# yuliangguo/OmniFusion

Hardware: AMD Instinct MI355X
Metric: panoramas/sec at 512x1024 ERP, N=18 256^2 patches; equi2pers+pers2equi GB/s vs HBM peak (higher is better)
Workload: dtype f16x3 (fp16 hi/lo pairs, fp32 accumulate: fp32-class); 1 GPU; cfg2/cfg4 shard: 8 panoramas/GPU/step, 512x1024 ERP, fov 80, nrows 4 (18 patches); full single-pass spherical_fusion forward (confidence=True) at patch size 128 — the only size the reference network exists at (SURVEY 0.1); random-init weights (seed 42); inputs resident in HBM; resample pair at 18x256^2 reported in roofline_resample; per_gpu_batch=8, global_batch=8, parallelism=image-sharded x1, execution=3 forwards in flight per GPU on 3 streams (spherical_fusion.pipelined)

## Files before the change

omnifusion_amd/csrc/omni_conv_sh.hip:

```cpp
#include "omni_conv_sh_common.h"

namespace {

__constant__ float wino_coef[16][4] = {
    {1, 0, 0, 0}, {1, 1, 0, 0}, {1, -1, 0, 0}, {0, -1, 0, 0},
    {1, 0, 1, 0}, {1, 1, 1, 1}, {1, -1, 1, -1}, {0, -1, 0, -1},
    {1, 0, -1, 0}, {1, 1, -1, -1}, {1, -1, -1, 1}, {0, -1, 0, 1},
    {0, 0, -1, 0}, {0, 0, -1, -1}, {0, 0, -1, 1}, {0, 0, 0, 1}};
template <int BM, int BN, int WM, int WN, int NST = 3, int NL = 0, bool PP = false, bool WINO = false, bool X1 = false>
__global__ __launch_bounds__(64 * (WM * WN + NL)) void conv_sh_kernel(ShConvArgs a)
{
    static_assert(!(WINO && X1), "Winograd: f16x3 only");
    static_assert(!PP || (NL > 0 && WM * WN == 8 && NST >= 3), "ping-pong: eight matrix waves (two per SIMD) + loader waves, three stages");
    static_assert(!WINO || (PP && BM / WM == 32 && BN / WN == 32), "Winograd: the ping-pong kernel with 32 x 32 wave tiles");
    constexpr int NW = WM * WN, LW = NL > 0 ? NL : NW, RPP = 8 * LW;
    constexpr int TM = BM / WM / 32, TN = BN / WN / 32;
    constexpr int APASS = BM / RPP, BPASS = BN / RPP, LPS = APASS + BPASS;
    static_assert(APASS >= 1 && BPASS >= 1, "a tile side must cover at least one DMA pass");
    constexpr int A_BYTES = BM * 128, STAGE = (BM + BN) * 128;
    __shared__ __attribute__((aligned(1024))) unsigned char lds[NST * STAGE];
    __shared__ long long cst[OMNI_ABL(32768) ? 256 : 1];
    const bool stamped = OMNI_ABL(32768) && blockIdx.x == 0 && blockIdx.y == 0 && a.ws != nullptr && a.splitk <= 1;
    auto cstamp = [&](int k) { if (OMNI_ABL(32768) && stamped && (threadIdx.x & 63) == 0 && k < 256) cst[k] = clock64(); };
    auto cdump = [&]() { if (OMNI_ABL(32768) && stamped && threadIdx.x == 0) for (int i = 0; i < 256; ++i) reinterpret_cast<long long*>(a.ws)[i] = cst[i]; };
// ... 633 lines not shown
    a.ws = ws;
    a.wt_major = omni_options().conv_wt_major == 2 || (omni_options().conv_wt_major == 1 &&
                 (long long)Cout * conv_sh_ksteps(a) * 128 > (long long)M * H * W * (C1 + C2) * 4) ? 1 : 0;
    a.post = post; a.post_rows = 1; a.wino_th = a.wino_tw = a.wino_pix = 0;
    if (post) {
        if (post_elems == 0 || post_elems % (size_t)Cout || post_elems / (size_t)Cout > 0x7fffffffull)
            OMNI_FAIL(OMNI_ERR_INVALID, "omni_conv2d_sh: the post-activation addend must hold whole rows of Cout channels");
        a.post_rows = (unsigned)(post_elems / (size_t)Cout);
    }
    hipStream_t s = (hipStream_t)stream;
    if (const int rc = conv_sh_launch(conv_sh_plan(a, fmt, post != nullptr, omni_options()), a, (fmt & 8) != 0, s); rc != OMNI_OK) return rc;
    OMNI_HIP(hipGetLastError());
    if (a.splitk > 1 && reduce) {
        const size_t n4 = (size_t)rows * Cout / 4;
        hipLaunchKernelGGL(sh_splitk_reduce_kernel, dim3((unsigned)((n4 + 255) / 256)), dim3(256), 0, s, (const float*)ws, bias, res, dst,
                           n4, Cout, a.splitk, (size_t)rows * Cout, act, a.dst_sh, a.res_f32);
        OMNI_HIP(hipGetLastError());
    }
    return OMNI_OK;
}

extern "C" int omni_conv2d_sh_plan(int fmt, int M, int H, int W, int C1, int C2, int Cout, int KH, int KW, int stride, int pad, int splitk, int has_post,
                                   int* out, int n_out)
{
    if (!out || n_out < 14) OMNI_FAIL(OMNI_ERR_INVALID, "omni_conv2d_sh_plan: needs room for 14 integers");
    ShConvArgs p{};
    if (const int rc = conv_sh_shape(p, M, H, W, C1, C2, Cout, KH, KW, stride, pad, splitk, has_post != 0); rc != OMNI_OK) return rc;
    const ConvShPlan q = conv_sh_plan(p, fmt, has_post != 0, omni_options());
    const int v[14] = {q.family, q.bm, q.bn, q.wm, q.wn, q.nst, q.nl, q.pp, q.th, q.iw, (int)q.grid_x, (int)q.grid_y, q.threads, p.splitk};
    std::copy(v, v + 14, out);
    return OMNI_OK;
}

extern "C" int omni_splitk_reduce_ln512(const float* parts, int nparts, const float* bias, const float* res, float* tok, const float* lg, const float* lb,
                                        float eps, void* y, int fmt, int rows, omni_stream_t stream)
{
    if (!parts || nparts < 1 || !tok || !lg || !lb || !y || rows <= 0) OMNI_FAIL(OMNI_ERR_INVALID, "omni_splitk_reduce_ln512: null pointer or empty input");
    hipStream_t s = (hipStream_t)stream;
    if (fmt & 1) hipLaunchKernelGGL(sh_splitk_reduce_ln512_kernel<true>, dim3((rows + 3) / 4), dim3(256), 0, s, parts, bias, res, tok, lg, lb, y, rows, nparts, (size_t)rows * 512, eps);
    else         hipLaunchKernelGGL(sh_splitk_reduce_ln512_kernel<false>, dim3((rows + 3) / 4), dim3(256), 0, s, parts, bias, res, tok, lg, lb, y, rows, nparts, (size_t)rows * 512, eps);
    OMNI_HIP(hipGetLastError());
    return OMNI_OK;
}

OMNI_SH_OVERFLOW_ACCESSOR(omni_sh_overflow_conv)

extern "C" int omni_sh_overflow(int* flag, int reset)
{
    if (!flag) OMNI_FAIL(OMNI_ERR_INVALID, "omni_sh_overflow: null output");
    OMNI_HIP(hipDeviceSynchronize());
    unsigned v = 0;
    if (omni_sh_overflow_conv(&v, reset) != 0 || omni_sh_overflow_halo(&v, reset) != 0 || omni_sh_overflow_up2(&v, reset) != 0 ||
        omni_sh_overflow_rows(&v, reset) != 0 || omni_sh_overflow_net(&v, reset) != 0 || omni_sh_overflow_pm(&v, reset) != 0 ||
        omni_sh_overflow_halo2(&v, reset) != 0 || omni_sh_overflow_up2_taps(&v, reset) != 0)
        OMNI_FAIL(OMNI_ERR_HIP, "omni_sh_overflow: could not read the device flag");
    *flag = v ? 1 : 0;
    return OMNI_OK;
}

extern "C" int omni_sh_from_f32(const float* src, void* dst, size_t n, omni_stream_t stream)
{
    if (!src || !dst || n % 32) OMNI_FAIL(OMNI_ERR_INVALID, "omni_sh_from_f32: null pointer or n % 32 != 0");
    if (n == 0) return OMNI_OK;
    hipLaunchKernelGGL(sh_from_f32_kernel, dim3((unsigned)((n / 4 + 255) / 256)), dim3(256), 0, (hipStream_t)stream, src, dst, n / 4);
    OMNI_HIP(hipGetLastError());
    return OMNI_OK;
}
extern "C" int omni_sh_to_f32(const void* src, float* dst, size_t n, omni_stream_t stream)
{
    if (!src || !dst || n % 32) OMNI_FAIL(OMNI_ERR_INVALID, "omni_sh_to_f32: null pointer or n % 32 != 0");
    if (n == 0) return OMNI_OK;
    hipLaunchKernelGGL(sh_to_f32_kernel, dim3((unsigned)((n / 4 + 255) / 256)), dim3(256), 0, (hipStream_t)stream, src, dst, n / 4);
    OMNI_HIP(hipGetLastError());
    return OMNI_OK;
}

namespace {

__global__ __launch_bounds__(256) void wino_input_sh_kernel(const void* __restrict__ src, void* __restrict__ V, int M, int H, int W, int C, size_t nt)
{
    const size_t i = (size_t)blockIdx.x * 256 + threadIdx.x;
    const int cq = C >> 2;
    if (i >= nt * cq) return;
    const size_t tl = i / cq;
    const int c = (int)(i - tl * cq) * 4;
    const int tw = W >> 1, th = H >> 1;
    const int m = (int)(tl / (size_t)(th * tw)), rem = (int)(tl - (size_t)m * th * tw), ty = rem / tw, tx = rem - ty * tw;
    f4v d[4][4];
#pragma unroll
    for (int a_ = 0; a_ < 4; ++a_)
#pragma unroll
        for (int b_ = 0; b_ < 4; ++b_) {
            const int y = 2 * ty - 1 + a_, x = 2 * tx - 1 + b_;
            d[a_][b_] = ((unsigned)y < (unsigned)H && (unsigned)x < (unsigned)W) ? act_load4<true>(src, (((size_t)m * H + y) * W + x) * C + c) : (f4v)(0.0f);
        }
    f4v u[4][4];
#pragma unroll
    for (int b_ = 0; b_ < 4; ++b_) { u[0][b_] = d[0][b_] - d[2][b_]; u[1][b_] = d[1][b_] + d[2][b_]; u[2][b_] = d[2][b_] - d[1][b_]; u[3][b_] = d[1][b_] - d[3][b_]; }
#pragma unroll
    for (int xi = 0; xi < 4; ++xi) {
        const f4v v0 = u[xi][0] - u[xi][2], v1 = u[xi][1] + u[xi][2], v2 = u[xi][2] - u[xi][1], v3 = u[xi][1] - u[xi][3];
        act_store4<true>(V, ((size_t)(4 * xi + 0) * nt + tl) * C + c, v0);
        act_store4<true>(V, ((size_t)(4 * xi + 1) * nt + tl) * C + c, v1);
        act_store4<true>(V, ((size_t)(4 * xi + 2) * nt + tl) * C + c, v2);
        act_store4<true>(V, ((size_t)(4 * xi + 3) * nt + tl) * C + c, v3);
    }
}
// ... 43 lines not shown
```

omnifusion_amd/csrc/omni_conv_sh_common.h:

```cpp
#pragma once
#include <stdlib.h>
#include <algorithm>
#include <type_traits>
#include "omni_internal.h"
#include "omni_sh.h"

#ifndef OMNI_CONV_ABL
#define OMNI_CONV_ABL 0
#endif
#define OMNI_ABL(bit) ((OMNI_CONV_ABL & (bit)) != 0)
#ifndef OMNI_PP_PRIO
#define OMNI_PP_PRIO 0
#endif
#ifndef OMNI_G1_PW
#define OMNI_G1_PW 4
#endif

namespace {

typedef float f16v __attribute__((ext_vector_type(16)));
typedef float f4v __attribute__((ext_vector_type(4)));
typedef _Float16 h8v __attribute__((ext_vector_type(8)));
typedef _Float16 h4v __attribute__((ext_vector_type(4)));
typedef _Float16 h2v __attribute__((ext_vector_type(2)));
// ... 152 lines not shown
            }
            if (a.act == OMNI_ACT_RELU) {
#pragma unroll
                for (int e = 0; e < 4; ++e) { v0[e] = fmaxf(v0[e], 0.f); v1[e] = fmaxf(v1[e], 0.f); }
            } else if (a.act == OMNI_ACT_GELU) {
#pragma unroll
                for (int e = 0; e < 4; ++e) { v0[e] = 0.5f * v0[e] * (1.0f + erff(v0[e] * 0.70710678118654752440f)); v1[e] = 0.5f * v1[e] * (1.0f + erff(v1[e] * 0.70710678118654752440f)); }
            }
            if (post) { v0 += pa[kk]; v1 += pb[kk]; }
            h4v h0, l0, h1, l1;
            sh_split4(v0, h0, l0); sh_split4(v1, h1, l1);
            h8v oh, ol;
#pragma unroll
            for (int e = 0; e < 4; ++e) { oh[e] = h0[e]; oh[4 + e] = h1[e]; ol[e] = l0[e]; ol[4 + e] = l1[e]; }
            *reinterpret_cast<h8v*>((unsigned char*)a.dst + off[kk]) = oh;
            *reinterpret_cast<h8v*>((unsigned char*)a.dst + off[kk] + 64) = ol;
        }
    }
}

__device__ __forceinline__ void splitk_finish(f4v v, size_t o, const float* __restrict__ bias, const void* __restrict__ res, void* __restrict__ dst,
                                              int Cout, int act, int dst_sh, int res_f32)
{
    if (bias) v += *reinterpret_cast<const f4v*>(bias + (o % Cout));
    if (res && res_f32) v += *reinterpret_cast<const f4v*>((const float*)res + o);
    else if (res) {
        const unsigned char* rp = (const unsigned char*)res + sh_off(o);
        v += sh_join4(*reinterpret_cast<const h4v*>(rp), *reinterpret_cast<const h4v*>(rp + 64));
    }
    if (act == OMNI_ACT_RELU) { v.x = fmaxf(v.x, 0.f); v.y = fmaxf(v.y, 0.f); v.z = fmaxf(v.z, 0.f); v.w = fmaxf(v.w, 0.f); }
    else if (act == OMNI_ACT_GELU) {
#pragma unroll
        for (int e = 0; e < 4; ++e) v[e] = 0.5f * v[e] * (1.0f + erff(v[e] * 0.70710678118654752440f));
    }
    if (dst_sh) {
        h4v hi, lo; sh_split4(v, hi, lo);
        unsigned char* dp = (unsigned char*)dst + sh_off(o);
        *reinterpret_cast<h4v*>(dp) = hi; *reinterpret_cast<h4v*>(dp + 64) = lo;
    } else {
        *reinterpret_cast<f4v*>((float*)dst + o) = v;
    }
}

constexpr int HT_W = 32, HPW = HT_W + 2;

}

int omni_halo_launch(const void* args, int bn, int th, bool up2, int iw, bool x1, unsigned grid, hipStream_t s);
int omni_conv_pm_launch(const void* args, int bn, bool x1, unsigned grid_x, unsigned grid_y, hipStream_t s);
int omni_sh_overflow_pm(unsigned* out, int reset);
int omni_halo2_launch(const void* args, int iw, bool x1, unsigned grid, hipStream_t s);
int omni_sh_overflow_halo2(unsigned* out, int reset);
int omni_sh_overflow_up2_taps(unsigned* out, int reset);
int omni_sh_overflow_halo(unsigned* out, int reset);
int omni_sh_overflow_up2(unsigned* out, int reset);
int omni_sh_overflow_rows(unsigned* out, int reset);
int omni_sh_overflow_net(unsigned* out, int reset);
```

omnifusion_amd/csrc/omni_conv_up2.hip:

```cpp
#include "omni_conv_sh_common.h"

namespace {

constexpr int HR_PITCH = 36;
struct HeadsArgs { const void* w16; float* hr; };

template <bool HEADS, bool X1 = false>
__global__ __launch_bounds__(HEADS ? 64 * (4 + OMNI_G1_PW) : 512) void conv3x3_up2_g1_kernel(ShConvArgs a, int ntiles, HeadsArgs hd)
{
    constexpr int BN = 32, TH = 4, NW = 4, RPP = 8 * NW;
    constexpr int PW = HEADS ? OMNI_G1_PW : 4, CPT = 32 / PW;
    constexpr int HPX = (TH + 2) * HPW, HA_INSTR = (HPX * 8 + 63) / 64, HA_BYTES = HA_INSTR * 1024;
    constexpr int BROWS = 3 * BN, BPASS = (BROWS + RPP - 1) / RPP, B_BYTES = BROWS * 128, W_OFF = 2 * HA_BYTES;
    __shared__ __attribute__((aligned(1024))) unsigned char lds[2 * HA_BYTES + 3 * B_BYTES];
    constexpr int ST_N = 40, ST_K = 5;
    __shared__ long long stamps[OMNI_ABL(32768) ? 2 * ST_N * ST_K : 1];
    auto stamp = [&](int who, int it, int k) { if (OMNI_ABL(32768) && blockIdx.x == 0 && it < ST_N && (threadIdx.x & 63) == 0) stamps[(who * ST_N + it) * ST_K + k] = clock64(); };

    const int t = threadIdx.x, lane = t & 63;
    const int wave = __builtin_amdgcn_readfirstlane(t >> 6);
    const bool consumer = wave < NW;
    const int tw = a.W / HT_W, th = a.H / TH, per_img = tw * th;
    const int xcd = blockIdx.x & 7, lb = blockIdx.x >> 3, nlb = gridDim.x >> 3;
    const int per = (ntiles + 7) >> 3, t_end = min(ntiles, (xcd + 1) * per);
// ... 271 lines not shown

extern "C" int omni_conv3x3_up2_sh_f16x3(const void* src, const void* wt16, const float* bias, void* dst, int fmt,
                                         int M, int Hl, int Wl, int C, int Cout, int act, omni_stream_t stream)
{
    if (!src || !wt16 || !dst) OMNI_FAIL(OMNI_ERR_INVALID, "omni_conv3x3_up2_sh: null pointer");
    if (M <= 0 || Hl <= 0 || Wl <= 0 || C <= 0 || C % 32 || Cout <= 0 || Cout % 32) OMNI_FAIL(OMNI_ERR_INVALID, "omni_conv3x3_up2_sh: bad shape (channels must be multiples of 32)");
    const int H = 2 * Hl, W = 2 * Wl;
    if (W % HT_W || H % 4) OMNI_FAIL(OMNI_ERR_UNSUPPORTED, "omni_conv3x3_up2_sh: the output must be a multiple of 4 rows x 32 columns");
    if ((long long)M * H * W >= (1ll << 31) || (long long)Cout * 9 * C * 4 >= (1ll << 31))
        OMNI_FAIL(OMNI_ERR_UNSUPPORTED, "omni_conv3x3_up2_sh: tensor too large for 32-bit indices");
    ShConvArgs a;
    a.src1 = src; a.src2 = nullptr; a.wt = wt16; a.bias = bias; a.res = nullptr; a.dst = dst; a.dst_sh = fmt & 1; a.res_f32 = 0;
    a.dbg = 0; a.noxcd = omni_options().conv_noxcd; a.wt_major = 0; a.epi_lds = omni_options().conv_epi_lds && !(fmt & 4);
#ifdef OMNI_DEBUG_BUILD
    a.dbg = omni_debug_bits("OMNI_CONV_DBG");
#endif
    a.M = M; a.H = H; a.W = W; a.C1 = C; a.C2 = 0; a.Cout = Cout; a.KH = 3; a.KW = 3; a.stride = 1; a.pad = 1; a.act = act;
    a.Ho = H; a.Wo = W; a.rows = M * H * W; a.splitk = 1; a.ws = nullptr; a.post = nullptr; a.post_rows = 1; a.wino_th = a.wino_tw = a.wino_pix = 0;
    const int grid = M * (H / 4) * (W / HT_W);
    const bool x1 = (fmt & 8) != 0;
    if (C == 32 && Cout == 32 && omni_options().conv_up2_persist) {
        const dim3 g1(grid < 256 ? (grid + 7) / 8 * 8 : 256);
        if (x1) hipLaunchKernelGGL((conv3x3_up2_g1_kernel<false, true>), g1, dim3(512), 0, (hipStream_t)stream, a, grid, HeadsArgs{nullptr, nullptr});
        else    hipLaunchKernelGGL(conv3x3_up2_g1_kernel<false>, g1, dim3(512), 0, (hipStream_t)stream, a, grid, HeadsArgs{nullptr, nullptr});
        OMNI_HIP(hipGetLastError());
        return OMNI_OK;
    }
    const bool bn64 = Cout % 64 == 0 && !((fmt & 4) && omni_options().conv_halo_up2_bn_lat == 32);
    const int bn = bn64 ? 64 : 32;
    if (const int rc = omni_halo_launch(&a, bn, 4, true, 0, x1, grid * (Cout / bn), (hipStream_t)stream); rc != OMNI_OK) return rc;
    OMNI_HIP(hipGetLastError());
    return OMNI_OK;
}

extern "C" size_t omni_up2_heads_scratch_bytes(int M, int P)
{
    if (M <= 0 || P <= 0 || P % 32) return 0;
    return (size_t)M * (P / 4) * (P / 32) * 4 * 6 * HR_PITCH * sizeof(float);
}
template <bool X1>
static int up2_heads_impl(const void* src, const void* wt16, const float* bias, const void* heads_w16f, float bias_pred, float bias_weight,
                          float* scratch, size_t scratch_bytes, float* out_a, float* out_c, int M, int P, int confidence, omni_stream_t stream)
{
    if (!src || !wt16 || !heads_w16f || !scratch || !out_a) OMNI_FAIL(OMNI_ERR_INVALID, "omni_conv3x3_up2_heads_sh: null pointer");
    if (M <= 0 || P <= 0 || P % 32) OMNI_FAIL(OMNI_ERR_INVALID, "omni_conv3x3_up2_heads_sh: the patch size must be a multiple of 32");
    if (scratch_bytes < omni_up2_heads_scratch_bytes(M, P)) OMNI_FAIL(OMNI_ERR_INVALID, "omni_conv3x3_up2_heads_sh: scratch too small (omni_up2_heads_scratch_bytes)");
    if ((long long)M * P * P >= (1ll << 31)) OMNI_FAIL(OMNI_ERR_UNSUPPORTED, "omni_conv3x3_up2_heads_sh: tensor too large for 32-bit indices");
    ShConvArgs a;
    a.src1 = src; a.src2 = nullptr; a.wt = wt16; a.bias = bias; a.res = nullptr; a.dst = nullptr; a.dst_sh = 0; a.res_f32 = 0;
    a.dbg = 0; a.noxcd = omni_options().conv_noxcd; a.wt_major = 0; a.epi_lds = 0;
    a.M = M; a.H = P; a.W = P; a.C1 = 32; a.C2 = 0; a.Cout = 32; a.KH = 3; a.KW = 3; a.stride = 1; a.pad = 1; a.act = OMNI_ACT_RELU;
    a.Ho = P; a.Wo = P; a.rows = M * P * P; a.splitk = 1; a.ws = nullptr; a.post = nullptr; a.post_rows = 1; a.wino_th = a.wino_tw = a.wino_pix = 0;
    const int grid = M * (P / 4) * (P / HT_W);
    hipLaunchKernelGGL((conv3x3_up2_g1_kernel<true, X1>), dim3(grid < 256 ? (grid + 7) / 8 * 8 : 256), dim3(64 * (4 + OMNI_G1_PW)), 0, (hipStream_t)stream, a, grid, HeadsArgs{heads_w16f, scratch});
    OMNI_HIP(hipGetLastError());
    const size_t n = (size_t)M * P * P / 4;
    hipLaunchKernelGGL(heads_finish_kernel, dim3((unsigned)((n + 255) / 256)), dim3(256), 0, (hipStream_t)stream, (const float*)scratch, bias_pred, bias_weight,
                       out_a, out_c, M, P, confidence);
    OMNI_HIP(hipGetLastError());
    return OMNI_OK;
}
extern "C" int omni_conv3x3_up2_heads_sh_f16x3(const void* src, const void* wt16, const float* bias, const void* heads_w16f, float bias_pred, float bias_weight,
                                               float* scratch, size_t scratch_bytes, float* out_a, float* out_c, int M, int P, int confidence, omni_stream_t stream)
{
    return up2_heads_impl<false>(src, wt16, bias, heads_w16f, bias_pred, bias_weight, scratch, scratch_bytes, out_a, out_c, M, P, confidence, stream);
}
extern "C" int omni_conv3x3_up2_heads_sh_f16x1(const void* src, const void* wt16, const float* bias, const void* heads_w16f, float bias_pred, float bias_weight,
                                               float* scratch, size_t scratch_bytes, float* out_a, float* out_c, int M, int P, int confidence, omni_stream_t stream)
{
    return up2_heads_impl<true>(src, wt16, bias, heads_w16f, bias_pred, bias_weight, scratch, scratch_bytes, out_a, out_c, M, P, confidence, stream);
}

extern "C" int omni_heads_pack_f16x3(const float* w_host, void* dst_host)
{
    if (!w_host || !dst_host) OMNI_FAIL(OMNI_ERR_INVALID, "omni_heads_pack: null pointer");
    _Float16* o = (_Float16*)dst_host;
    for (int kc = 0; kc < 2; ++kc)
        for (int lane = 0; lane < 64; ++lane)
            for (int e = 0; e < 8; ++e) {
                const int r = lane & 31, h = lane >> 5, g = r >> 3, hh = (r >> 2) & 1, dxi = r & 3;
                float w = 0.0f;
                if (g < 3 && dxi < 3) {
                    const int pair = g + 3 * hh, dy = pair / 2, head = pair % 2, ch = 16 * kc + 8 * (e >> 2) + 4 * h + (e & 3);
                    w = w_host[(head * 9 + dy * 3 + dxi) * 32 + ch];
                }
                const _Float16 hi = (w < 6.103515625e-05f && w > -6.103515625e-05f) ? (_Float16)0.0f : (_Float16)w;
                o[(kc * 64 + lane) * 8 + e] = hi;
                o[((2 + kc) * 64 + lane) * 8 + e] = (_Float16)((w - (float)hi) * 2048.0f);
            }
    return OMNI_OK;
}
```

omnifusion_amd/csrc/omni_geometry.hip:

```cpp
#include <math.h>
#include <stdlib.h>
#include <string.h>
#include <mutex>
#include <vector>
#include <memory>

#include "omni_internal.h"

static thread_local std::string g_err;
void omni_set_error(const std::string& msg) { g_err = msg; }
extern "C" const char* omni_last_error(void) { return g_err.c_str(); }
extern "C" int omni_version(void) { return OMNI_VERSION; }

namespace {
struct OptName { const char* name; const char* env; int OmniOptions::* field; int dflt; };
const OptName kOpts[] = {
    {"conv_sh_tile", "OMNI_CONV_SH_TILE", &OmniOptions::conv_sh_tile, -1},
    {"conv_nohalo", "OMNI_CONV_NOHALO", &OmniOptions::conv_nohalo, 0},
    {"conv_halo_th", "OMNI_CONV_HALO_TH", &OmniOptions::conv_halo_th, 4},
    {"conv_big_blocks", "OMNI_CONV_BIG_BLOCKS", &OmniOptions::conv_big_blocks, 128},
    {"conv_halo_bn_lat", "OMNI_CONV_HALO_BN_LAT", &OmniOptions::conv_halo_bn_lat, 32},
    {"conv_deep_loaders", "OMNI_CONV_DEEP_LOADERS", &OmniOptions::conv_deep_loaders, 1},
    {"conv_halo_up2_bn_lat", "OMNI_CONV_HALO_UP2_BN_LAT", &OmniOptions::conv_halo_up2_bn_lat, 64},
    {"conv_halo_bn", "OMNI_CONV_HALO_BN", &OmniOptions::conv_halo_bn, 64},
    {"conv_img", "OMNI_CONV_IMG", &OmniOptions::conv_img, 1},
    {"conv_nodeep", "OMNI_CONV_NODEEP", &OmniOptions::conv_nodeep, 0},
    {"conv_pingpong", "OMNI_CONV_PINGPONG", &OmniOptions::conv_pingpong, 1},
    {"conv_pm", "OMNI_CONV_PM", &OmniOptions::conv_pm, 1},
    {"conv_noxcd", "OMNI_CONV_NOXCD", &OmniOptions::conv_noxcd, 0},
    {"conv_wt_major", "OMNI_CONV_WT_MAJOR", &OmniOptions::conv_wt_major, 1},
    {"conv_stem_pc", "OMNI_CONV_STEM_PC", &OmniOptions::conv_stem_pc, 1},
    {"conv_epi_lds", "OMNI_CONV_EPI_LDS", &OmniOptions::conv_epi_lds, 1},
    {"conv_up2_persist", "OMNI_CONV_UP2_PERSIST", &OmniOptions::conv_up2_persist, 1},
    {"splitk_max", "OMNI_SPLITK_MAX", &OmniOptions::splitk_max, 0},
    {"e2p_gather", "OMNI_E2P_GATHER", &OmniOptions::e2p_gather, 0},
    {"e2p_notab", "OMNI_E2P_NOTAB", &OmniOptions::e2p_notab, 0},
    {"e2p_verbose", "OMNI_E2P_VERBOSE", &OmniOptions::e2p_verbose, 0},
    {"e2p_bwd_simple", "OMNI_E2P_BWD_SIMPLE", &OmniOptions::e2p_bwd_simple, 0},
    {"p2e_bwd_simple", "OMNI_P2E_BWD_SIMPLE", &OmniOptions::p2e_bwd_simple, 0},
    {"bwd_table_mb", "OMNI_BWD_TABLE_MB", &OmniOptions::bwd_table_mb, 1024},
    {"bwd_wide", "OMNI_BWD_WIDE", &OmniOptions::bwd_wide, 1},
    {"bwd_lmax", "OMNI_BWD_LMAX", &OmniOptions::bwd_lmax, 0},
    {"bwd_chunk", "OMNI_BWD_CHUNK", &OmniOptions::bwd_chunk, 0},
    {"p2e_gather", "OMNI_P2E_GATHER", &OmniOptions::p2e_gather, 0},
    {"e2p_nbuf", "OMNI_E2P_NBUF", &OmniOptions::e2p_nbuf, 0},
    {"e2p_slot_kb", "OMNI_E2P_SLOT_KB", &OmniOptions::e2p_slot_kb, 6},
    {"e2p_tile_h", "OMNI_E2P_TILE_H", &OmniOptions::e2p_tile_h, 0},
    {"e2p_ref_lds", "OMNI_E2P_REF_LDS", &OmniOptions::e2p_ref_lds, 1},
    {"e2p_store", "OMNI_E2P_STORE", &OmniOptions::e2p_store, 1},
    {"e2p_slots", "OMNI_E2P_SLOTS", &OmniOptions::e2p_slots, 0},
    {"e2p_split", "OMNI_E2P_SPLIT", &OmniOptions::e2p_split, 0},
    {"e2p_full", "OMNI_E2P_FULL", &OmniOptions::e2p_full, -1},
    {"e2p_fb_planes", "OMNI_E2P_FB_PLANES", &OmniOptions::e2p_fb_planes, 0},
    {"e2p_fb_pos", "OMNI_E2P_FB_POS", &OmniOptions::e2p_fb_pos, 0},
    {"e2p_region", "OMNI_E2P_REGION", &OmniOptions::e2p_region, 0},
    {"p2e_band", "OMNI_P2E_BAND", &OmniOptions::p2e_band, 0},
    {"p2e_nbuf", "OMNI_P2E_NBUF", &OmniOptions::p2e_nbuf, 0},
    {"p2e_lds_kb", "OMNI_P2E_LDS_KB", &OmniOptions::p2e_lds_kb, 0},
    {"p2e_planes", "OMNI_P2E_PLANES", &OmniOptions::p2e_planes, 0},
    {"p2e_walk", "OMNI_P2E_WALK", &OmniOptions::p2e_walk, 1},
    {"p2e_tile8", "OMNI_P2E_TILE8", &OmniOptions::p2e_tile8, 1},
    {"p2e_store", "OMNI_P2E_STORE", &OmniOptions::p2e_store, 1},
    {"fv_bwd_lds", "OMNI_FV_BWD_LDS", &OmniOptions::fv_bwd_lds, 1},
    {"geom_cache_max", "OMNI_GEOM_CACHE_MAX", &OmniOptions::geom_cache_max, 16},
    {"chamfer_split", "OMNI_CHAMFER_SPLIT", &OmniOptions::chamfer_split, 1},
    {"augment_lut", "OMNI_AUGMENT_LUT", &OmniOptions::augment_lut, 1},
    {"conv_halo2", "OMNI_CONV_HALO2", &OmniOptions::conv_halo2, 1},
    {"conv_wgrad_rows", "OMNI_CONV_WGRAD_ROWS", &OmniOptions::conv_wgrad_rows, 0},
};
}

OmniOptions& omni_options()
{
    static OmniOptions o = [] {
        OmniOptions v;
        for (const OptName& k : kOpts) {
            const char* e = getenv(k.env);
            v.*(k.field) = e ? (*e ? atoi(e) : 1) : k.dflt;
        }
        return v;
    }();
    return o;
}

int omni_num_cus()
{
// ... 250 lines not shown
```

omnifusion_amd/csrc/omni_internal.h:

```cpp
#pragma once
#include <mutex>
#include <hip/hip_runtime.h>
#include <hip/hip_fp16.h>
#include <stdint.h>
#include <string>
#include <vector>

#include "../../include/omnifusion.h"

#define OMNI_MAX_PATCH 46
#define OMNI_WAVE 64

void omni_set_error(const std::string& msg);
#define OMNI_FAIL(code, msg) do { omni_set_error(msg); return (code); } while (0)
#define OMNI_HIP(expr) do { hipError_t e_ = (expr); if (e_ != hipSuccess) {                   \
        omni_set_error(std::string(#expr) + ": " + hipGetErrorString(e_)); return OMNI_ERR_HIP; } } while (0)

struct OmniOptions {
    int conv_sh_tile;
    int conv_nohalo;
    int conv_halo_th;
    int conv_halo_bn_lat;
    int conv_halo_up2_bn_lat;
    int conv_deep_loaders;
    int conv_big_blocks;
    int conv_halo_bn;
    int conv_img;
    int conv_nodeep;
    int conv_pingpong;
    int conv_pm;
    int conv_noxcd;
    int conv_wt_major;
    int conv_stem_pc;
    int conv_epi_lds;
    int conv_up2_persist;
    int splitk_max;
    int e2p_gather;
    int e2p_notab;
    int e2p_verbose;
    int e2p_bwd_simple;
    int p2e_bwd_simple;
    int p2e_gather;
    int e2p_nbuf;
    int e2p_store;
    int e2p_slots;
    int e2p_split;
    int e2p_full;
    int e2p_fb_planes;
    int e2p_region;
    int e2p_fb_pos;
    int e2p_ref_lds;
    int e2p_tile_h;
    int e2p_slot_kb;
    int p2e_band;
    int p2e_lds_kb;
    int p2e_nbuf;
    int p2e_planes;
    int p2e_store;
    int p2e_tile8;
    int p2e_walk;
    int bwd_wide;
    int bwd_chunk;
    int bwd_lmax;
    int bwd_table_mb;
    int fv_bwd_lds;
    int geom_cache_max;
    int chamfer_split;
    int augment_lut;
    int conv_halo2;
    int conv_wgrad_rows;
};
OmniOptions& omni_options();
int omni_num_cus();

#ifdef OMNI_DEBUG_BUILD
#define OMNI_DBG(a, bit) (((a).dbg & (bit)) != 0)
int omni_debug_bits(const char* env_name);
long long* omni_debug_trace_buf();
#else
#define OMNI_DBG(a, bit) false
#endif

struct PatchTab {
    int   N;
    float lam0[OMNI_MAX_PATCH];
    float slam[OMNI_MAX_PATCH];
    float clam[OMNI_MAX_PATCH];
    float sphi[OMNI_MAX_PATCH];
// ... 94 lines not shown
```

omnifusion_amd/isa.py:

```python
import os
import re
import subprocess
import sys
import tempfile

LLVM = os.environ.get("OMNI_LLVM_BIN", "/opt/rocm/lib/llvm/bin")
TARGET = "hipv4-amdgcn-amd-amdhsa--gfx950"
FORBIDDEN = re.compile(r"\bv_pk_(mul|add|fma)_f32\b")
COUNTED = ("e2p_box_kernel", "p2e_lds_kernel", "p2e_walk_kernel", "e2p_ref_kernel", "up2_taps_fused_kernel")
HOT = ("conv_sh_kernel", "conv3x3_halo_sh_kernel", "conv3x3_up2_g1_kernel", "stem_f16x3_pc_kernel", "heads_kernel", "maxpool_kernel",
       "layernorm512_kernel", "attention_kernel", "upsample_sh8_kernel", "halo2_sh_kernel")
HOST_ONLY = ("omni_png.o", "omni_geometry.o")


def _device_object(obj, tmp):
    fat = os.path.join(tmp, "fat.bin")
    co = os.path.join(tmp, "dev.co")
    r = subprocess.run([os.path.join(LLVM, "llvm-objcopy"), "--dump-section", f".hip_fatbin={fat}", obj, os.path.join(tmp, "copy.o")],
                       stderr=subprocess.DEVNULL)
    if r.returncode != 0 or not os.path.exists(fat) or os.path.getsize(fat) == 0:
        return None
    subprocess.check_call([os.path.join(LLVM, "clang-offload-bundler"), "--unbundle", "--type=o", f"--input={fat}",
                           f"--targets={TARGET}", f"--output={co}"])
    return co


def disassemble(obj):
    with tempfile.TemporaryDirectory() as tmp:
        co = _device_object(obj, tmp)
        if co is None:
            return ""
        return subprocess.check_output([os.path.join(LLVM, "llvm-objdump"), "-d", "--mcpu=gfx950", co]).decode()


def kernel_meta(obj):
    with tempfile.TemporaryDirectory() as tmp:
        co = _device_object(obj, tmp)
        if co is None:
            return []
        txt = subprocess.check_output([os.path.join(LLVM, "llvm-readelf"), "--notes", co]).decode()
    out, cur = [], None
    keys = {".vgpr_count": "vgpr", ".agpr_count": "agpr", ".sgpr_count": "sgpr", ".group_segment_fixed_size": "lds",
            ".private_segment_fixed_size": "scratch", ".vgpr_spill_count": "vgpr_spill", ".sgpr_spill_count": "sgpr_spill",
            ".name": "name"}
    for line in txt.splitlines():
        m = re.match(r"^  - \.(\w+):\s*(\S+)\s*$", line)
        if m:
            cur = {}
            out.append(cur)
            line = "    ." + m.group(1) + ": " + m.group(2)
        m = re.match(r"^    (\.\w+):\s*(\S+)\s*$", line)
        if m and cur is not None and m.group(1) in keys:
            v = m.group(2)
            cur[keys[m.group(1)]] = v if m.group(1) == ".name" else int(v)
    return [k for k in out if "name" in k]


def demangle(names):
    try:
        p = subprocess.run([os.path.join(LLVM, "llvm-cxxfilt")], input="\n".join(names).encode(), stdout=subprocess.PIPE, check=True)
        return p.stdout.decode().splitlines()
    except Exception:
# ... 70 lines not shown
```

Baseline: 4475 panoramas/s.

## Add persistent tap-first up2 conv+heads kernel computing conv before upsampling

Adds a new persistent kernel for the final upsample-by-2 3x3 conv plus prediction heads at patch size 128. It applies each 3x3 tap's channel mix at the low 64x64 resolution with MFMA, then does the bilinear upsample separably (vertical, then horizontal) through LDS. The heads 1x1 projection is fused on the parked output. This aims to cut the conv arithmetic by doing the matmuls at a quarter of the pixels, at the cost of a complex LDS schedule, many barriers, and a one-block-per-CU occupancy. The path is on by default through a new option and falls back to the old kernel when pointers are misaligned or the size is not 128.

```diff
diff --git a/omnifusion_amd/csrc/omni_conv_sh.hip b/omnifusion_amd/csrc/omni_conv_sh.hip
--- a/omnifusion_amd/csrc/omni_conv_sh.hip
+++ b/omnifusion_amd/csrc/omni_conv_sh.hip
@@ -709,7 +709,8 @@
     unsigned v = 0;
     if (omni_sh_overflow_conv(&v, reset) != 0 || omni_sh_overflow_halo(&v, reset) != 0 || omni_sh_overflow_up2(&v, reset) != 0 ||
         omni_sh_overflow_rows(&v, reset) != 0 || omni_sh_overflow_net(&v, reset) != 0 || omni_sh_overflow_pm(&v, reset) != 0 ||
-        omni_sh_overflow_halo2(&v, reset) != 0 || omni_sh_overflow_up2_taps(&v, reset) != 0)
+        omni_sh_overflow_halo2(&v, reset) != 0 || omni_sh_overflow_up2_taps(&v, reset) != 0 ||
+        omni_sh_overflow_up2_heads_taps(&v, reset) != 0)
         OMNI_FAIL(OMNI_ERR_HIP, "omni_sh_overflow: could not read the device flag");
     *flag = v ? 1 : 0;
     return OMNI_OK;
diff --git a/omnifusion_amd/csrc/omni_conv_sh_common.h b/omnifusion_amd/csrc/omni_conv_sh_common.h
--- a/omnifusion_amd/csrc/omni_conv_sh_common.h
+++ b/omnifusion_amd/csrc/omni_conv_sh_common.h
@@ -228,6 +228,8 @@
 int omni_halo2_launch(const void* args, int iw, bool x1, unsigned grid, hipStream_t s);
 int omni_sh_overflow_halo2(unsigned* out, int reset);
 int omni_sh_overflow_up2_taps(unsigned* out, int reset);
+int omni_up2_heads_taps_launch(const void* src, const void* wt16, const float* bias, const void* heads_w16f, float* hr, int M, hipStream_t s);
+int omni_sh_overflow_up2_heads_taps(unsigned* out, int reset);
 int omni_sh_overflow_halo(unsigned* out, int reset);
 int omni_sh_overflow_up2(unsigned* out, int reset);
 int omni_sh_overflow_rows(unsigned* out, int reset);
diff --git a/omnifusion_amd/csrc/omni_conv_up2.hip b/omnifusion_amd/csrc/omni_conv_up2.hip
--- a/omnifusion_amd/csrc/omni_conv_up2.hip
+++ b/omnifusion_amd/csrc/omni_conv_up2.hip
@@ -347,8 +347,14 @@
     a.M = M; a.H = P; a.W = P; a.C1 = 32; a.C2 = 0; a.Cout = 32; a.KH = 3; a.KW = 3; a.stride = 1; a.pad = 1; a.act = OMNI_ACT_RELU;
     a.Ho = P; a.Wo = P; a.rows = M * P * P; a.splitk = 1; a.ws = nullptr; a.post = nullptr; a.post_rows = 1; a.wino_th = a.wino_tw = a.wino_pix = 0;
     const int grid = M * (P / 4) * (P / HT_W);
-    hipLaunchKernelGGL((conv3x3_up2_g1_kernel<true, X1>), dim3(grid < 256 ? (grid + 7) / 8 * 8 : 256), dim3(64 * (4 + OMNI_G1_PW)), 0, (hipStream_t)stream, a, grid, HeadsArgs{heads_w16f, scratch});
-    OMNI_HIP(hipGetLastError());
+    const bool taps = !X1 && P == 128 && omni_options().conv_up2_heads_taps == 1 &&
+                      !((uintptr_t)src % 16 || (uintptr_t)wt16 % 16 || (uintptr_t)bias % 16 || (uintptr_t)heads_w16f % 16 || (uintptr_t)scratch % 16);
+    if (taps) {
+        if (const int rc = omni_up2_heads_taps_launch(src, wt16, bias, heads_w16f, scratch, M, (hipStream_t)stream); rc != OMNI_OK) return rc;
+    } else {
+        hipLaunchKernelGGL((conv3x3_up2_g1_kernel<true, X1>), dim3(grid < 256 ? (grid + 7) / 8 * 8 : 256), dim3(64 * (4 + OMNI_G1_PW)), 0, (hipStream_t)stream, a, grid, HeadsArgs{heads_w16f, scratch});
+        OMNI_HIP(hipGetLastError());
+    }
     const size_t n = (size_t)M * P * P / 4;
     hipLaunchKernelGGL(heads_finish_kernel, dim3((unsigned)((n + 255) / 256)), dim3(256), 0, (hipStream_t)stream, (const float*)scratch, bias_pred, bias_weight,
                        out_a, out_c, M, P, confidence);
diff --git a/omnifusion_amd/csrc/omni_conv_up2_heads_taps.hip b/omnifusion_amd/csrc/omni_conv_up2_heads_taps.hip
--- /dev/null
+++ b/omnifusion_amd/csrc/omni_conv_up2_heads_taps.hip
@@ -0,0 +1,287 @@
+#include <stdint.h>
+#include "omni_conv_sh_common.h"
+
+namespace {
+
+constexpr int HR_PITCH = 36;
+
+struct HeadsTapsArgs {
+    const void* src;
+    const void* wt;
+    const float* bias;
+    const void* hw16;
+    float* hr;
+    int nbands;
+};
+
+constexpr int WL = 64, HL = 64, ROWS = 4, SROWS = ROWS + 2, NPX = SROWS * WL, NF = NPX / 32;
+constexpr int TAP_BYTES = 32 * 128, W_BYTES = 9 * TAP_BYTES, CH_BYTES = NPX * 128, ROW_BYTES = WL * 128;
+constexpr int BANDS_PER_IMG = HL / ROWS;
+
+__host__ __device__ constexpr int tap_at(int s) { return 3 * (s % 3) + s / 3; }
+
+__global__ __launch_bounds__(512, 1) void up2_heads_taps_kernel(HeadsTapsArgs a)
+{
+    __shared__ __attribute__((aligned(1024))) unsigned char lds[W_BYTES + 2 * CH_BYTES];
+    static_assert(sizeof(lds) <= 160 * 1024 && NF == 12 && 4 * 128 * 128 <= 2 * CH_BYTES, "one block per CU; half a band's SH rows fit the two chunks");
+
+    const int t = threadIdx.x, lane = t & 63;
+    const int wave = __builtin_amdgcn_readfirstlane(t >> 6);
+    const int xcd = blockIdx.x & 7, lb = blockIdx.x >> 3, nlb = gridDim.x >> 3;
+    const int per = (a.nbands + 7) >> 3, b_end = min(a.nbands, (xcd + 1) * per);
+    int bandid = xcd * per + lb;
+    if (bandid >= b_end) return;
+
+    {
+        const rsrc_t rsw = make_rsrc(a.wt, (size_t)32 * 9 * 128);
+#pragma unroll
+        for (int k = 0; k < 5; ++k) {
+            const int n = wave + 8 * k;
+            if (n < 36) {
+                const int tp = n >> 2, d = (n & 3) * 4 + (lane >> 4), pw = (lane & 15) ^ d, row = 2 * d + (pw >> 3);
+                dma16(rsw, lds + n * 1024, ((row * 9 + tp) * 8 + (pw & 7)) * 16, 0);
+            }
+        }
+    }
+    const int wfo = ((lane & 31) >> 1) * 256 + ((((lane & 1) * 8 + (lane >> 5)) ^ ((lane & 31) >> 1)) * 16);
+
+    auto frag = [&](int fi) { return fi == 0 || wave >= 4 ? wave : wave + 8; };
+    h8v xh[2][2], xl[2][2];
+    auto load_x = [&](int bid) {
+        const int m = bid / BANDS_PER_IMG, sbase = (bid - m * BANDS_PER_IMG) * ROWS - 1;
+#pragma unroll
+        for (int fi = 0; fi < 2; ++fi) {
+            const int p = frag(fi) * 32 + (lane & 31), sr = p / WL, cx = p - sr * WL;
+            const int row = min(max(sbase + sr, 0), HL - 1);
+            const unsigned char* sp = (const unsigned char*)a.src + ((size_t)(m * HL + row) * WL + cx) * 128 + (lane >> 5) * 16;
+#pragma unroll
+            for (int kc = 0; kc < 2; ++kc) {
+                xh[fi][kc] = *reinterpret_cast<const h8v*>(sp + kc * 32);
+                xl[fi][kc] = *reinterpret_cast<const h8v*>(sp + 64 + kc * 32);
+            }
+        }
+    };
+    load_x(bandid);
+
+    const int quad = t & 7, j = t >> 3;
+    auto col_off = [&](int col) { return col * 128 + ((quad ^ ((col >> 1) & 3)) * 16); };
+    const int coff1 = col_off(j);
+    wait_vm<0>();
+    __builtin_amdgcn_s_barrier();
+    asm volatile("" ::: "memory");
+
+    for (;;) {
+        const int m = bandid / BANDS_PER_IMG, band = bandid - m * BANDS_PER_IMG;
+        const int r0 = band * ROWS, sbase = r0 - 1;
+        const int next = bandid + nlb;
+        const bool top = r0 == 0, bot = r0 + ROWS - 1 == HL - 1;
+        const float hy0[4] = {top ? 0.0f : 0.75f, top ? 1.0f : 0.25f, 0.75f, 0.25f}, ly0[4] = {top ? 0.0f : 0.25f, top ? 0.0f : 0.75f, 0.25f, 0.75f};
+        const float hy3 = bot ? 0.0f : 0.25f, ly3 = bot ? 0.0f : 0.75f;
+
+        f4v out[ROWS][2][2];
+        f4v S[ROWS][2];
+
+        auto tap = [&]<int s>() {
+            constexpr int tp = tap_at(s), ky = tp / 3, kx = tp - 3 * ky;
+            unsigned char* chunk = lds + W_BYTES + (s & 1) * CH_BYTES;
+            {
+                const unsigned char* wb = lds + tp * TAP_BYTES;
+                h8v wh[2], wl[2];
+#pragma unroll
+                for (int kc = 0; kc < 2; ++kc) {
+                    wh[kc] = *reinterpret_cast<const h8v*>(wb + (wfo ^ (2 * kc * 16)));
+                    wl[kc] = *reinterpret_cast<const h8v*>(wb + (wfo ^ ((2 * kc + 4) * 16)));
+                }
+#pragma unroll
+                for (int fi = 0; fi < 2; ++fi) {
+                    if (fi == 1 && wave >= 4) break;
+                    f16v acc = (f16v)(0.0f), acc1 = (f16v)(0.0f);
+#pragma unroll
+                    for (int kc = 0; kc < 2; ++kc) {
+                        acc  = __builtin_amdgcn_mfma_f32_32x32x16_f16(wh[kc], xh[fi][kc], acc, 0, 0, 0);
+                        acc1 = __builtin_amdgcn_mfma_f32_32x32x16_f16(wl[kc], xh[fi][kc], acc1, 0, 0, 0);
+                        acc1 = __builtin_amdgcn_mfma_f32_32x32x16_f16(wh[kc], xl[fi][kc], acc1, 0, 0, 0);
+                    }
+                    const int px = frag(fi) * 32 + (lane & 31);
+                    unsigned char* cp = chunk + px * 128;
+                    const int sw = (px >> 1) & 3;
+#pragma unroll
+                    for (int q = 0; q < 4; ++q) {
+                        f4v v;
+#pragma unroll
+                        for (int e = 0; e < 4; ++e) v[e] = acc_join<false>(acc1[4 * q + e], acc[4 * q + e]);
+                        *reinterpret_cast<f4v*>(cp + (((2 * q + (lane >> 5)) ^ sw) * 16)) = v;
+                    }
+                    __builtin_amdgcn_sched_barrier(0);
+                }
+            }
+            if constexpr (s == 8) load_x(next < b_end ? next : bandid);
+            wait_lds_reads();
+            __builtin_amdgcn_s_barrier();
+            asm volatile("" ::: "memory");
+            {
+                constexpr int klo = ky >> 1, khi = ROWS + ((ky + 1) >> 1);
+                f4v R[ROWS + 2];
+#pragma unroll
+                for (int k = klo; k <= khi; ++k)
+                    R[k] = *reinterpret_cast<const f4v*>(chunk + (min(max(r0 - 1 + k, 0), HL - 1) - sbase) * ROW_BYTES + coff1);
+#pragma unroll
+                for (int it = 0; it < ROWS; ++it)
+#pragma unroll
+                    for (int ay = 0; ay < 2; ++ay) {
+                        const int uy = ay + ky, r = uy >> 1;
+                        const float h = it == 0 ? hy0[uy] : it == ROWS - 1 && uy == 3 ? hy3 : (uy & 1) ? 0.25f : 0.75f;
+                        const float l = it == 0 ? ly0[uy] : it == ROWS - 1 && uy == 3 ? ly3 : (uy & 1) ? 0.75f : 0.25f;
+                        f4v v;
+                        if constexpr (ky != 0) v = S[it][ay];
+#pragma unroll
+                        for (int e = 0; e < 4; ++e)
+                            if constexpr (ky == 0) v[e] = fmaf(l, R[it + r + 1][e], h * R[it + r][e]);
+                            else v[e] = fmaf(l, R[it + r + 1][e], fmaf(h, R[it + r][e], v[e]));
+                        asm volatile("" : "+v"(v));
+                        S[it][ay] = v;
+                    }
+                __builtin_amdgcn_sched_barrier(0);
+            }
+            if constexpr (ky == 2) {
+                unsigned char* other = lds + W_BYTES + ((s & 1) ^ 1) * CH_BYTES;
+                auto horizontal = [&]<int ay>(const unsigned char* buf) {
+                    int jj = j;
+                    asm volatile("" : "+v"(jj));
+                    const int coff[3] = {col_off(max(jj - 1, 0)), 0, col_off(min(jj + 1, WL - 1))};
+                    float hx[4], lx[4];
+                    hx[0] = jj > 0 ? 0.75f : 0.0f;      lx[0] = jj > 0 ? 0.25f : 0.0f;
+                    hx[1] = jj > 0 ? 0.25f : 1.0f;      lx[1] = jj > 0 ? 0.75f : 0.0f;
+                    hx[2] = 0.75f;                      lx[2] = 0.25f;
+                    hx[3] = jj < WL - 1 ? 0.25f : 0.0f; lx[3] = jj < WL - 1 ? 0.75f : 0.0f;
+#pragma unroll
+                    for (int it = 0; it < ROWS; ++it) {
+                        const unsigned char* rp = buf + it * ROW_BYTES;
+                        const f4v own = S[it][ay];
+                        f4v left = own, right = own;
+                        if (kx <= 1) left = *reinterpret_cast<const f4v*>(rp + coff[0]);
+                        if (kx >= 1) right = *reinterpret_cast<const f4v*>(rp + coff[2]);
+#pragma unroll
+                        for (int bx = 0; bx < 2; ++bx) {
+                            const int ux = bx + kx, c = ux >> 1;
+                            const f4v va = c == 0 ? left : own, vb = c == 0 ? own : right;
+                            f4v o;
+                            if constexpr (kx != 0) o = out[it][ay][bx];
+#pragma unroll
+                            for (int e = 0; e < 4; ++e)
+                                if constexpr (kx == 0) o[e] = fmaf(lx[ux], vb[e], hx[ux] * va[e]);
+                                else o[e] = fmaf(lx[ux], vb[e], fmaf(hx[ux], va[e], o[e]));
+                            asm volatile("" : "+v"(o));
+                            out[it][ay][bx] = o;
+                        }
+                    }
+                    __builtin_amdgcn_sched_barrier(0);
+                };
+#pragma unroll
+                for (int it = 0; it < ROWS; ++it) *reinterpret_cast<f4v*>(other + it * ROW_BYTES + coff1) = S[it][0];
+                wait_lds_reads();
+                __builtin_amdgcn_s_barrier();
+                asm volatile("" ::: "memory");
+#pragma unroll
+                for (int it = 0; it < ROWS; ++it) *reinterpret_cast<f4v*>(chunk + it * ROW_BYTES + coff1) = S[it][1];
+                __builtin_amdgcn_sched_barrier(0);
+                horizontal.template operator()<0>(other);
+                wait_lds_reads();
+                __builtin_amdgcn_s_barrier();
+                asm volatile("" ::: "memory");
+                horizontal.template operator()<1>(chunk);
+            }
+        };
+        tap.template operator()<0>(); tap.template operator()<1>(); tap.template operator()<2>();
+        tap.template operator()<3>(); tap.template operator()<4>(); tap.template operator()<5>();
+        tap.template operator()<6>(); tap.template operator()<7>(); tap.template operator()<8>();
+
+        h8v hwf[4];
+#pragma unroll
+        for (int k = 0; k < 4; ++k) hwf[k] = *reinterpret_cast<const h8v*>((const unsigned char*)a.hw16 + k * 1024 + lane * 16);
+        unsigned char* park = lds + W_BYTES;
+        const int pk_piece = 2 * (quad >> 2) + (quad & 1), pk_half = ((quad >> 1) & 1) * 8;
+        const f4v bv = a.bias ? *reinterpret_cast<const f4v*>(a.bias + quad * 4) : (f4v)(0.0f);
+#pragma unroll
+        for (int half = 0; half < 2; ++half) {
+            wait_lds_reads();
+            __builtin_amdgcn_s_barrier();
+            asm volatile("" ::: "memory");
+#pragma unroll
+            for (int itl = 0; itl < 2; ++itl)
+#pragma unroll
+                for (int ay = 0; ay < 2; ++ay)
+#pragma unroll
+                    for (int bx = 0; bx < 2; ++bx) {
+                        f4v o = out[2 * half + itl][ay][bx] + bv;
+                        o.x = fmaxf(o.x, 0.f); o.y = fmaxf(o.y, 0.f); o.z = fmaxf(o.z, 0.f); o.w = fmaxf(o.w, 0.f);
+                        h4v hi, lo; sh_split4(o, hi, lo);
+                        const int p = (2 * itl + ay) * 128 + 2 * j + bx, d = p >> 1;
+                        unsigned char* pp = park + d * 256 + pk_half;
+                        *reinterpret_cast<h4v*>(pp + ((((p & 1) * 8 + pk_piece) ^ (d & 15)) * 16)) = hi;
+                        *reinterpret_cast<h4v*>(pp + ((((p & 1) * 8 + pk_piece + 4) ^ (d & 15)) * 16)) = lo;
+                    }
+            wait_lds_reads();
+            __builtin_amdgcn_s_barrier();
+            asm volatile("" ::: "memory");
+#pragma unroll
+            for (int sg = 0; sg < 2; ++sg) {
+                const int seg = wave + 8 * sg, row = seg >> 2, sx = seg & 3;
+                const int px = lane & 31, h = lane >> 5;
+                const int p = row * 128 + sx * 32 + px, d = p >> 1;
+                const unsigned char* fp = park + d * 256;
+                const int fo = (((p & 1) * 8 + h) ^ (d & 15)) * 16;
+                h8v ph[2], pl[2];
+#pragma unroll
+                for (int kc = 0; kc < 2; ++kc) {
+                    ph[kc] = *reinterpret_cast<const h8v*>(fp + (fo ^ (2 * kc * 16)));
+                    pl[kc] = *reinterpret_cast<const h8v*>(fp + (fo ^ ((2 * kc + 4) * 16)));
+                }
+                f16v d0 = (f16v)(0.0f), d1 = (f16v)(0.0f);
+#pragma unroll
+                for (int kc = 0; kc < 2; ++kc) {
+                    d0 = __builtin_amdgcn_mfma_f32_32x32x16_f16(hwf[kc], ph[kc], d0, 0, 0, 0);
+                    d1 = __builtin_amdgcn_mfma_f32_32x32x16_f16(hwf[2 + kc], ph[kc], d1, 0, 0, 0);
+                    d1 = __builtin_amdgcn_mfma_f32_32x32x16_f16(hwf[kc], pl[kc], d1, 0, 0, 0);
+                }
+                const size_t tile = ((size_t)m * (2 * BANDS_PER_IMG) + 2 * band + half) * 4 + sx;
+                float* hp = a.hr + (tile * 4 + row) * (6 * HR_PITCH);
+#pragma unroll
+                for (int g = 0; g < 3; ++g) {
+                    const float tl = fmaf(d1[4 * g], 4.8828125e-4f, d0[4 * g]), tc = fmaf(d1[4 * g + 1], 4.8828125e-4f, d0[4 * g + 1]),
+                                tr = fmaf(d1[4 * g + 2], 4.8828125e-4f, d0[4 * g + 2]);
+                    const float fl = __shfl_up(tl, 1, 32), fr = __shfl_down(tr, 1, 32);
+                    const float sum = ((px > 0 ? fl : 0.0f) + tc) + (px < 31 ? fr : 0.0f);
+                    float* rowp = hp + (g + 3 * h) * HR_PITCH;
+                    rowp[px] = sum;
+                    if (px == 0) rowp[32] = tr;
+                    if (px == 31) rowp[33] = tl;
+                }
+            }
+        }
+        if (next >= b_end) break;
+        bandid = next;
+        wait_lds_reads();
+        __builtin_amdgcn_s_barrier();
+        asm volatile("" ::: "memory");
+    }
+}
+
+}
+
+OMNI_SH_OVERFLOW_ACCESSOR(omni_sh_overflow_up2_heads_taps)
+
+int omni_up2_heads_taps_launch(const void* src, const void* wt16, const float* bias, const void* heads_w16f, float* hr, int M, hipStream_t s)
+{
+    if (!src || !wt16 || !heads_w16f || !hr || M <= 0) OMNI_FAIL(OMNI_ERR_INVALID, "omni_up2_heads_taps_launch: null pointer or no patches");
+    if ((uintptr_t)src % 16 || (uintptr_t)wt16 % 16 || (uintptr_t)bias % 16 || (uintptr_t)heads_w16f % 16 || (uintptr_t)hr % 16)
+        OMNI_FAIL(OMNI_ERR_INVALID, "omni_up2_heads_taps_launch: tensors must be 16-byte aligned");
+    if ((long long)M * HL * WL >= (1ll << 31)) OMNI_FAIL(OMNI_ERR_UNSUPPORTED, "omni_up2_heads_taps_launch: tensor too large for 32-bit indices");
+    HeadsTapsArgs a;
+    a.src = src; a.wt = wt16; a.bias = bias; a.hw16 = heads_w16f; a.hr = hr; a.nbands = M * BANDS_PER_IMG;
+    const int cus = omni_num_cus() / 8 * 8;
+    const unsigned grid = (unsigned)(a.nbands < cus ? (a.nbands + 7) / 8 * 8 : cus);
+    hipLaunchKernelGGL(up2_heads_taps_kernel, dim3(grid), dim3(512), 0, s, a);
+    OMNI_HIP(hipGetLastError());
+    return OMNI_OK;
+}
diff --git a/omnifusion_amd/csrc/omni_geometry.hip b/omnifusion_amd/csrc/omni_geometry.hip
--- a/omnifusion_amd/csrc/omni_geometry.hip
+++ b/omnifusion_amd/csrc/omni_geometry.hip
@@ -32,6 +32,7 @@
     {"conv_stem_pc", "OMNI_CONV_STEM_PC", &OmniOptions::conv_stem_pc, 1},
     {"conv_epi_lds", "OMNI_CONV_EPI_LDS", &OmniOptions::conv_epi_lds, 1},
     {"conv_up2_persist", "OMNI_CONV_UP2_PERSIST", &OmniOptions::conv_up2_persist, 1},
+    {"conv_up2_heads_taps", "OMNI_CONV_UP2_HEADS_TAPS", &OmniOptions::conv_up2_heads_taps, 1},
     {"splitk_max", "OMNI_SPLITK_MAX", &OmniOptions::splitk_max, 0},
     {"e2p_gather", "OMNI_E2P_GATHER", &OmniOptions::e2p_gather, 0},
     {"e2p_notab", "OMNI_E2P_NOTAB", &OmniOptions::e2p_notab, 0},
diff --git a/omnifusion_amd/csrc/omni_internal.h b/omnifusion_amd/csrc/omni_internal.h
--- a/omnifusion_amd/csrc/omni_internal.h
+++ b/omnifusion_amd/csrc/omni_internal.h
@@ -34,6 +34,7 @@
     int conv_stem_pc;
     int conv_epi_lds;
     int conv_up2_persist;
+    int conv_up2_heads_taps;
     int splitk_max;
     int e2p_gather;
     int e2p_notab;
diff --git a/omnifusion_amd/isa.py b/omnifusion_amd/isa.py
--- a/omnifusion_amd/isa.py
+++ b/omnifusion_amd/isa.py
@@ -7,7 +7,7 @@
 LLVM = os.environ.get("OMNI_LLVM_BIN", "/opt/rocm/lib/llvm/bin")
 TARGET = "hipv4-amdgcn-amd-amdhsa--gfx950"
 FORBIDDEN = re.compile(r"\bv_pk_(mul|add|fma)_f32\b")
-COUNTED = ("e2p_box_kernel", "p2e_lds_kernel", "p2e_walk_kernel", "e2p_ref_kernel", "up2_taps_fused_kernel")
+COUNTED = ("e2p_box_kernel", "p2e_lds_kernel", "p2e_walk_kernel", "e2p_ref_kernel", "up2_taps_fused_kernel", "up2_heads_taps_kernel")
 HOT = ("conv_sh_kernel", "conv3x3_halo_sh_kernel", "conv3x3_up2_g1_kernel", "stem_f16x3_pc_kernel", "heads_kernel", "maxpool_kernel",
        "layernorm512_kernel", "attention_kernel", "upsample_sh8_kernel", "halo2_sh_kernel")
 HOST_ONLY = ("omni_png.o", "omni_geometry.o")
```

After: 4587 panoramas/s, median of 6. 1.03x the previous value.
